# hkust-vgd/scanobjectnn

Hardware: NVIDIA H100
Metric: point-clouds/sec (B=32, N=2048, 15-class) (higher is better)
Workload: dtype f32

## Files before the change

scanobjectnn_b200/csrc/tc_mlp.cu:

```cuda
#include <float.h>
#include <stdlib.h>

#include <atomic>
#include <type_traits>

#include "common.cuh"
#include "mlp_internal.cuh"
#include "tc_common.cuh"

namespace psa {

using namespace tc;

constexpr int kMaxTcLayers = 2;


struct TcArgs {
    long long groups;
    int K;
    int n, m;
    const float* xyz;
    const float* new_xyz;
    const float* uf;
    const int* idx;
// ... 798 lines not shown
                for (int w = 1; w < wpg; ++w) mx = fmaxf(mx, s_red[0][grp * wpg + w][cl]);
                const long long wg = rs / a.pool_k;
                if (!big) {
                    a.out[(size_t)wg * a.N + nt * Nt + cl] = mx;
                } else {
                    int code = __float_as_int(mx);
                    code = code >= 0 ? code : code ^ 0x7fffffff;
                    atomicMax(reinterpret_cast<int*>(a.out) + (size_t)wg * a.N + nt * Nt + cl, code);
                }
            }
            unit_bar_sync(1, kDenseConsumers);
        }
    }
    if constexpr (NP == 2) {
        if (f16x2_overflowed(ovf) || (tid == 0 && a.wflag != nullptr && *a.wflag != 0u)) atomicOr(a.ovf, 1u);
    }
}

bool tc_dense_eligible(long long rows, int K, int N, int pool_k) {
    if (rows < 128 || K < 32 || N < 64 || (N % 64) != 0) return false;
    if (N > 64 && (N % 128) != 0) return false;
    if (!(pool_k == 1 || pool_k == 32 || pool_k == 64 || (pool_k >= 128 && pool_k % 128 == 0))) return false;
    if (pool_k > 1 && rows % pool_k != 0) return false;
    return true;
}

static std::atomic<int> g_tc_np{2};
int tc_np() { return g_tc_np; }

static size_t tc_dense_image_off3(int K, int N) { return tc_image_alloc_bytes((K + 63) & ~63, N, 2); }
size_t tc_dense_image_bytes(int K, int N) { return tc_dense_image_off3(K, N) + tc_image_alloc_bytes((K + 63) & ~63, N, 3); }

static size_t tc_plan_image_bytes(int Kp, int N) { return g_tc_np == 2 ? tc_image_alloc_bytes(Kp, N, 2) + tc_image_alloc_bytes(Kp, N, 3) : tc_image_alloc_bytes(Kp, N, 3); }

int tc_dense_nt(long long rows, int N) {
    const bool wide = (N % 128) == 0 && 2 * ((rows + 127) / 128 * (N / 128)) > kNumSMs;
    return (wide ? 128 : 64) | image_flag(g_tc_np);
}

int build_image(int K, int Kp, int N, int Nt, const float* W, uint8_t* image, cudaStream_t st, const unsigned int* run_if) {
    if (Nt & kImageF16x2) {
        unsigned int* trailer = reinterpret_cast<unsigned int*>(image + tc_image_trailer_off(Kp, N, 2));
        float* colscale = reinterpret_cast<float*>(image + tc_image_colscale_off(Kp, N, 2));
        PSA_CUDA(cudaMemsetAsync(trailer, 0, 256, st));
        tc_col_scale_kernel<<<(N + 31) / 32, dim3(32, 8), 0, st>>>(K, N, W, colscale, trailer);
        int rc = check_launch("tc_col_scale_kernel");
        if (rc != PSA_OK) return rc;
        tc_prep_weights_kernel<2><<<(Kp * N + 255) / 256, 256, 0, st>>>(K, Kp, N, Nt & ~kImageFlags, W, colscale, image, run_if);
    } else {
        tc_prep_weights_kernel<3><<<(Kp * N + 255) / 256, 256, 0, st>>>(K, Kp, N, Nt & ~kImageFlags, W, nullptr, image, run_if);
    }
    return check_launch("tc_prep_weights_kernel");
}
const unsigned int* image_trailer(const uint8_t* image, int Kp, int N) {
    return reinterpret_cast<const unsigned int*>(image + tc_image_trailer_off(Kp, N, 2));
}
const float* image_colscale(const uint8_t* image, int Kp, int N) {
    return reinterpret_cast<const float*>(image + tc_image_colscale_off(Kp, N, 2));
}

template <int NP, int NC>
static int launch_tc_dense_shape(const TcDenseArgs& a, cudaStream_t st) {
    const size_t smem = (size_t)dense_stages(NP, NC) * dense_stage_bytes(NP, NC) + 1024;
    PSA_CUDA(cudaFuncSetAttribute(tc_dense_kernel<NP, NC>, cudaFuncAttributeMaxDynamicSharedMemorySize, (int)smem));
    int dev = 0, sms = 0, per_sm = 0;
    PSA_CUDA(cudaGetDevice(&dev));
    PSA_CUDA(cudaDeviceGetAttribute(&sms, cudaDevAttrMultiProcessorCount, dev));
    PSA_CUDA(cudaOccupancyMaxActiveBlocksPerMultiprocessor(&per_sm, tc_dense_kernel<NP, NC>, kDenseThreads, smem));
    const long long tiles = (a.rows + 127) / 128 * (a.N / (64 * NC)), resident = (long long)sms * (per_sm > 0 ? per_sm : 1);
    tc_dense_kernel<NP, NC><<<(unsigned)(tiles < resident ? tiles : resident), kDenseThreads, smem, st>>>(a);
    return check_launch("tc_dense_kernel");
}

template <int NP>
static int launch_tc_dense_np(TcDenseArgs& a, int Nt, cudaStream_t st) {
    const bool big = a.pool_k > 128;
    if (big) { int rc0 = launch_fill_ord_neg_inf(a.rows / a.pool_k * a.N, a.out, st, a.run_if); if (rc0 != PSA_OK) return rc0; }
    const int rc = Nt == 128 ? launch_tc_dense_shape<NP, 2>(a, st) : launch_tc_dense_shape<NP, 1>(a, st);
    if (rc != PSA_OK) return rc;
    if (big) return launch_decode_ord(a.rows / a.pool_k * a.N, a.out, st, a.run_if);
    return PSA_OK;
}

constexpr int kTileCounterWords = PSA_MAX_MLP_LAYERS;

static int launch_tc_dense_rerun(TcDenseArgs a, int Nt, const float* W, const uint8_t* prebuilt, uint8_t* ws_img, const unsigned int* run_if,
                                 unsigned int* counter, cudaStream_t st) {
    uint8_t* img3 = ws_img + tc_dense_image_off3(a.K, a.N);
    if (prebuilt != nullptr) {
        img3 = const_cast<uint8_t*>(prebuilt) + tc_image_alloc_bytes(a.Kp, a.N, 2);
    } else {
        const int rc = build_image(a.K, a.Kp, a.N, Nt | kImageBf16x3, W, img3, st, run_if);
        if (rc != PSA_OK) return rc;
    }
    a.image = img3; a.ovf = nullptr; a.wflag = nullptr; a.colscale = nullptr; a.run_if = run_if; a.tile_counter = counter;
    return launch_tc_dense_np<3>(a, Nt, st);
}

int launch_tc_dense(long long rows, int K, int N, int pool_k, int relu, const float* x, const float* W, const float* scale,
                    const float* shift, float* out, const uint8_t* prebuilt, uint8_t* ws_img, unsigned int* flag, unsigned int* counters,
                    cudaStream_t st, const float* xyz3 = nullptr, const float* w3 = nullptr, const float* group_add = nullptr,
                    long long group_rows = 0) {
    const int Kp = (K + 63) & ~63;
    const int Nt = tc_dense_nt(rows, N) & ~kImageFlags;
    TcDenseArgs a;
    a.rows = rows; a.K = K; a.Kp = Kp; a.N = N; a.pool_k = pool_k; a.relu = relu;
    a.x = x; a.scale = scale; a.shift = shift; a.out = out; a.xyz3 = xyz3; a.w3 = w3;
    a.group_add = group_add; a.group_rows = group_rows;
    a.tile_counter = counters;
    uint8_t* img3 = ws_img + tc_dense_image_off3(K, N);
    int rc;
    if (g_tc_np == 3) {
        if (prebuilt == nullptr) { rc = build_image(K, Kp, N, Nt | kImageBf16x3, W, img3, st); if (rc != PSA_OK) return rc; }
        a.image = prebuilt ? prebuilt : img3;
        return launch_tc_dense_np<3>(a, Nt, st);
    }
    if (prebuilt == nullptr) { rc = build_image(K, Kp, N, Nt | kImageF16x2, W, ws_img, st); if (rc != PSA_OK) return rc; }
    a.image = prebuilt ? prebuilt : ws_img;
    a.ovf = flag; a.wflag = image_trailer(a.image, Kp, N); a.colscale = image_colscale(a.image, Kp, N);
    rc = launch_tc_dense_np<2>(a, Nt, st);
    if (rc != PSA_OK) return rc;
    return launch_tc_dense_rerun(a, Nt, W, prebuilt, ws_img, flag, counters + 1, st);
}

bool tc_train_fwd_eligible(long long rows, int K, int N) {
    return rows >= 128 && K >= 128 && K <= 512 && N >= 128 && (N % 128) == 0;
}
int launch_tc_dense_train(long long rows, int K, int N, const float* x, const float* in_scale, const float* in_shift, int in_relu,
                          const float* W, const float* bias, float* y, float* stat_partial, uint8_t* image_ws, cudaStream_t st) {
    const int Kp = (K + 63) & ~63;
    int rc = build_image(K, Kp, N, 128 | kImageBf16x3, W, image_ws, st);
    if (rc != PSA_OK) return rc;
    TcDenseArgs a;
    a.rows = rows; a.K = K; a.Kp = Kp; a.N = N; a.pool_k = 1; a.relu = 0;
    a.x = x; a.image = image_ws; a.scale = nullptr; a.shift = bias; a.out = y; a.xyz3 = nullptr; a.w3 = nullptr;
    a.in_scale = in_scale; a.in_shift = in_shift; a.in_relu = in_relu; a.stat_partial = stat_partial;
    return launch_tc_dense_np<3>(a, 128, st);
}

static const uint8_t* prebuilt_image(const psa_mlp* mlp, int l, int row0, int Nt) {
    if (mlp->image[l] != nullptr && mlp->image_nt[l] == Nt && mlp->image_row0[l] == row0) return reinterpret_cast<const uint8_t*>(mlp->image[l]);
    return nullptr;
}

bool tc_sa_eligible(const psa_mlp* mlp, int c, int nsample, TcArgs* out, int np) {
    if (mlp->n_layers < 2 || mlp->n_layers > 1 + kMaxTcLayers) return false;
    if (!(nsample == 32 || nsample == 64 || nsample == 128)) return false;
    if (mlp->channels[0] != 3 + c) return false;
    const int C1 = mlp->channels[1];
    if (!(C1 == 64 || C1 == 128)) return false;
    TcArgs a{};
    a.C1 = C1;
    a.nl = mlp->n_layers - 1;
    a.np = np;
    for (int l = 0; l < a.nl; ++l) {
        a.Kd[l] = mlp->channels[1 + l];
        a.Ntot[l] = mlp->channels[2 + l];
        if (!(a.Kd[l] == 64 || a.Kd[l] == 128)) return false;
        const bool is_last = (l == a.nl - 1);
        if (!is_last && !(a.Ntot[l] == 64 || a.Ntot[l] == 128)) return false;
        if (is_last && !(a.Ntot[l] == 64 || a.Ntot[l] % 128 == 0)) return false;
    }
    a.stream_last = 0;
    if (tc_sa_layout(a).total + 1024 > kSmemBudget) a.stream_last = 1;
    if (tc_sa_layout(a).total + 1024 > kSmemBudget) return false;
    *out = a;
    return true;
}
bool tc_sa_eligible(const psa_mlp* mlp, int c, int nsample, TcArgs* out) {
    TcArgs a3;
    if (!tc_sa_eligible(mlp, c, nsample, &a3, 3)) return false;
    if (g_tc_np == 3) { *out = a3; return true; }
    return tc_sa_eligible(mlp, c, nsample, out, 2);
}

size_t tc_sa_workspace_bytes(const TcArgs& a, int b, int n, int c) {
    size_t bytes = 256;
    for (int l = 0; l < a.nl; ++l) bytes += tc_image_alloc_bytes(a.Kd[l], a.Ntot[l], 2) + tc_image_alloc_bytes(a.Kd[l], a.Ntot[l], 3);
    if (c > 0) bytes += (((size_t)b * n * a.C1 * sizeof(float) + 255) & ~(size_t)255) + tc_dense_image_bytes(c, a.C1);
    return bytes;
}

static int tc_sa_image_nt() { return kSaNt | image_flag(g_tc_np); }

template <int NP, int C1, int NL, int N0>
static int launch_tc_sa_shape(const TcArgs& a, long long ctas_needed, size_t smem, cudaStream_t st) {
    PSA_CUDA(cudaFuncSetAttribute(tc_sa_kernel<NP, C1, NL, N0>, cudaFuncAttributeMaxDynamicSharedMemorySize, (int)smem));
    int dev = 0, sms = 0, per_sm = 0;
    PSA_CUDA(cudaGetDevice(&dev));
    PSA_CUDA(cudaDeviceGetAttribute(&sms, cudaDevAttrMultiProcessorCount, dev));
    PSA_CUDA(cudaOccupancyMaxActiveBlocksPerMultiprocessor(&per_sm, tc_sa_kernel<NP, C1, NL, N0>, kSaThreads, smem));
    const long long resident = (long long)sms * (per_sm > 0 ? per_sm : 1);
    const int ctas = (int)(ctas_needed < 1 ? 1 : ctas_needed < resident ? ctas_needed : resident);
    tc_sa_kernel<NP, C1, NL, N0><<<ctas, kSaThreads, smem, st>>>(a);
    return check_launch("tc_sa_kernel");
}

template <int NP>
static int launch_tc_sa_np(TcArgs& a, cudaStream_t st) {
    const uint32_t limit = 223u * 1024u;
    a.joint = a.K == 128 || a.stream_last;
    if (!a.joint && tc_sa_layout(a).total + 1024 + sa_carry_bytes(a) + sa_red_bytes(1) > limit) a.joint = 1;
    const size_t used = (size_t)tc_sa_layout(a).total + 1024 + sa_carry_bytes(a);
    const int ncl = a.Ntot[a.nl - 1] / 64;
    a.pool_chunks = 1;
    if (!a.stream_last)
        for (int ng = ncl; ng > 1; --ng)
            if (ncl % ng == 0 && used + sa_red_bytes(ng) <= limit) { a.pool_chunks = ng; break; }
    const int C = sa_chunk(a.K, a.joint);
    const long long nchunks = (a.groups + C - 1) / C;
    const long long ctas_needed = a.joint ? nchunks : (nchunks + 1) / 2;
    const size_t smem = used + sa_red_bytes(a.pool_chunks);
    if (a.nl == 1) return a.C1 == 64 ? launch_tc_sa_shape<NP, 64, 1, 0>(a, ctas_needed, smem, st) : launch_tc_sa_shape<NP, 128, 1, 0>(a, ctas_needed, smem, st);
    if (a.C1 == 64) return a.Ntot[0] == 64 ? launch_tc_sa_shape<NP, 64, 2, 64>(a, ctas_needed, smem, st) : launch_tc_sa_shape<NP, 64, 2, 128>(a, ctas_needed, smem, st);
    return a.Ntot[0] == 64 ? launch_tc_sa_shape<NP, 128, 2, 64>(a, ctas_needed, smem, st) : launch_tc_sa_shape<NP, 128, 2, 128>(a, ctas_needed, smem, st);
}

static int tc_sa_run(TcArgs& a, int b, int n, int m, int c, int nsample, const float* xyz, const float* new_xyz, const float* points,
                     const int* idx, const psa_mlp* mlp, const float* w1c, float* out, void* workspace, cudaStream_t st) {
    int rc = PSA_OK;
    uint8_t* ws = reinterpret_cast<uint8_t*>(workspace);
    unsigned int* words = reinterpret_cast<unsigned int*>(ws);
    PSA_CUDA(cudaMemsetAsync(ws, 0, 256, st));
    ws += 256;
    uint8_t* img2[kMaxTcLayers];
    uint8_t* img3[kMaxTcLayers];
    for (int l = 0; l < a.nl; ++l) {
        img2[l] = ws; ws += tc_image_alloc_bytes(a.Kd[l], a.Ntot[l], 2);
        img3[l] = ws; ws += tc_image_alloc_bytes(a.Kd[l], a.Ntot[l], 3);
    }
    const float* uf = nullptr;
    if (c > 0) {
        float* ufw = reinterpret_cast<float*>(ws);
        uint8_t* uimg = ws + (((size_t)b * n * a.C1 * sizeof(float) + 255) & ~(size_t)255);
        const float* w1f = mlp->weight[0] + (size_t)3 * a.C1;
        if (tc_dense_eligible((long long)b * n, c, a.C1, 1)) {
            rc = launch_tc_dense((long long)b * n, c, a.C1, 1, 0, points, w1f, nullptr, nullptr, ufw, prebuilt_image(mlp, 0, 3, tc_dense_nt((long long)b * n, a.C1)),
                                 uimg, words + 3, words + 4, st);
        } else {
            DenseArgs d;
            d.rows = (long long)b * n; d.K = c; d.N = a.C1; d.pool_k = 1; d.relu = 0;
            d.x = points; d.W = w1f; d.scale = nullptr; d.shift = nullptr; d.out = ufw;
            rc = launch_dense(d, st);
        }
        if (rc != PSA_OK) return rc;
        uf = ufw;
    }
    auto fill = [&](TcArgs& t) {
        t.groups = (long long)b * m; t.K = nsample; t.n = n; t.m = m;
        t.xyz = xyz; t.new_xyz = new_xyz; t.idx = idx; t.out = out; t.uf = uf;
        t.w1x = mlp->weight[0]; t.s1 = mlp->scale[0]; t.t1 = mlp->shift[0]; t.relu1 = mlp->relu[0];
        t.ovf = nullptr; t.run_if = nullptr; t.w1c = w1c;
        for (int l = 0; l < t.nl; ++l) {
            t.s[l] = mlp->scale[1 + l]; t.t[l] = mlp->shift[1 + l]; t.relu[l] = mlp->relu[1 + l]; t.wflag[l] = nullptr; t.colscale[l] = nullptr;
        }
    };
    fill(a);
    for (int l = 0; l < a.nl; ++l) {
        const int nt_img = tc_sa_image_nt();
        const uint8_t* pre = prebuilt_image(mlp, 1 + l, 0, nt_img);
        uint8_t* own = a.np == 2 ? img2[l] : img3[l];
        if (pre == nullptr) { rc = build_image(a.Kd[l], a.Kd[l], a.Ntot[l], nt_img, mlp->weight[1 + l], own, st); if (rc != PSA_OK) return rc; }
        a.image[l] = pre ? pre : own;
        if (a.np == 2) { a.wflag[l] = image_trailer(a.image[l], a.Kd[l], a.Ntot[l]); a.colscale[l] = image_colscale(a.image[l], a.Kd[l], a.Ntot[l]); }
    }
    a.tile_counter = words;
    if (a.np == 3) return launch_tc_sa_np<3>(a, st);
    a.ovf = words + 2;
    rc = launch_tc_sa_np<2>(a, st);
    if (rc != PSA_OK) return rc;
    TcArgs a3;
    PSA_REQUIRE(tc_sa_eligible(mlp, c, nsample, &a3, 3), "sa_module: internal error (bf16x3 eligibility)");
    fill(a3);
    for (int l = 0; l < a3.nl; ++l) {
        const uint8_t* pre = prebuilt_image(mlp, 1 + l, 0, kSaNt | kImageF16x2);
        if (pre != nullptr) {
            a3.image[l] = pre + tc_image_alloc_bytes(a3.Kd[l], a3.Ntot[l], 2);
        } else {
            rc = build_image(a3.Kd[l], a3.Kd[l], a3.Ntot[l], kSaNt | kImageBf16x3, mlp->weight[1 + l], img3[l], st, words + 2);
            if (rc != PSA_OK) return rc;
            a3.image[l] = img3[l];
        }
    }
    a3.tile_counter = words + 1;
    a3.run_if = words + 2;
    return launch_tc_sa_np<3>(a3, st);
}

struct TcGroupAllArgs {
    int c;
    int N[3];
    int Nt[3];
    const float* points;
    const float* xyz;
    const float* w3;
    const uint8_t* image[3];
    const float* colscale[3];
    const unsigned int* wflag[3];
    const float* scale[3];
    const float* shift[3];
    int relu[3];
    float* out;
    unsigned int* ovf;
};

constexpr int kGaStages = 3;
constexpr uint32_t kGaStageBytes = 32768u;
constexpr uint32_t kGaSmemBudget = 222u * 1024u;
__host__ __device__ inline uint32_t group_all_smem(int W0, int W1, int W2) {
    return 1024u + kGaStages * kGaStageBytes + (uint32_t)(W0 + W1) / 64u * kDenseXBytes + 12u * (uint32_t)(W0 + W1 + W2);
}

__device__ __forceinline__ uint32_t cluster_ctarank() {
    uint32_t r;
    asm volatile("mov.u32 %0, %%cluster_ctarank;\n" : "=r"(r));
    return r;
}
__device__ __forceinline__ uint32_t mapa_shared(uint32_t addr, uint32_t rank) {
    uint32_t r;
    asm volatile("mapa.shared::cluster.u32 %0, %1, %2;\n" : "=r"(r) : "r"(addr), "r"(rank));
    return r;
}
__device__ __forceinline__ float2 ld_cluster_f32x2(uint32_t addr) {
    float2 v;
    asm volatile("ld.shared::cluster.v2.f32 {%0, %1}, [%2];\n" : "=f"(v.x), "=f"(v.y) : "r"(addr) : "memory");
    return v;
}
__device__ __forceinline__ void cluster_sync_all() {
    asm volatile("barrier.cluster.arrive.release.aligned;\n\tbarrier.cluster.wait.acquire.aligned;\n" ::: "memory");
}
__device__ __forceinline__ void mbar_arrive_cluster(uint32_t addr) {
    asm volatile("fence.acq_rel.cluster;\n\tmbarrier.arrive.release.cluster.shared::cluster.b64 _, [%0];\n" ::"r"(addr) : "memory");
}
__device__ __forceinline__ void mbar_wait_cluster(uint64_t* bar, uint32_t parity) {
    uint32_t done;
    const uint32_t addr = smem_u32(bar);
    do {
        asm volatile(
            "{\n\t.reg .pred p;\n\t"
            "mbarrier.try_wait.parity.acquire.cluster.shared::cta.b64 p, [%1], %2;\n\t"
            "selp.u32 %0, 1, 0, p;\n\t}\n"
            : "=r"(done)
            : "r"(addr), "r"(parity)
            : "memory");
    } while (!done);
}

template <int NC0, int NC1>
__global__ void __cluster_dims__(4, 1, 1) __launch_bounds__(kDenseThreads, 1)
tc_group_all_kernel(const __grid_constant__ TcGroupAllArgs a) {
    constexpr int NP = 2, S = kGaStages;
    constexpr uint32_t piece = 8192u, chunk = 16384u;
    extern __shared__ uint8_t smem_raw[];
    __shared__ __align__(8) uint64_t s_full[S], s_empty[S], s_ready[2], s_done;
    __shared__ float s_red[8][128];
    const int tid = threadIdx.x, lane = tid & 31, warp = tid >> 5;
    const uint32_t rank = cluster_ctarank();
    const int cloud = blockIdx.x >> 2;
    uint8_t* base = smem_raw + ((1024u - (smem_u32(smem_raw) & 1023u)) & 1023u);
    constexpr int W0 = 64 * NC0, W1 = 64 * NC1;
    const int W2 = a.N[2] / 4;
    uint8_t* slice0 = base + S * kGaStageBytes;
    uint8_t* slice1 = slice0 + NC0 * kDenseXBytes;
    float* aff0 = reinterpret_cast<float*>(slice1 + NC1 * kDenseXBytes);
    float* aff1 = aff0 + 3 * W0;
    float* aff2 = aff1 + 3 * W1;
    {
        float* aff[3] = {aff0, aff1, aff2};
        const int W[3] = {W0, W1, W2};
#pragma unroll
        for (int l = 0; l < 3; ++l)
            for (int i = tid; i < W[l]; i += kDenseThreads) {
                const int col = (int)rank * W[l] + i;
                const float cs = __ldg(a.colscale[l] + col);
                aff[l][i] = (a.scale[l] ? __ldg(a.scale[l] + col) : 1.f) * cs;
                aff[l][W[l] + i] = a.shift[l] ? __ldg(a.shift[l] + col) : 0.f;
                aff[l][2 * W[l] + i] = pow2_rcp(cs);
            }
    }
    if (tid == 0) {
        for (int i = 0; i < S; ++i) { mbar_init(&s_full[i], 1); mbar_init(&s_empty[i], kDenseConsumers / 32); }
        mbar_init(&s_ready[0], 4); mbar_init(&s_ready[1], 4); mbar_init(&s_done, 4);
        fence_mbar_init();
    }
    __syncthreads();
    cluster_sync_all();
    const int KC[3] = {a.c / 64, 4 * W0 / 64, 4 * W1 / 64};

    if (warp >= kDenseConsumers / 32) {
        asm volatile("setmaxnreg.dec.sync.aligned.u32 40;\n");
        if (warp != kDenseConsumers / 32) return;
        uint32_t u = 0;
#pragma unroll
        for (int l = 0; l < 3; ++l) {
            const int pw = l == 0 ? W0 : l == 1 ? W1 : 128, passes = l == 2 ? W2 / 128 : 1, Nt = a.Nt[l];
            for (int p = 0; p < passes; ++p) {
                const int j0 = ((int)rank * (l == 0 ? W0 : l == 1 ? W1 : W2) + p * pw) / 64;
                for (int kb = 0; kb < KC[l]; ++kb, ++u) {
                    const int s = (int)(u % S);
                    if (u >= (uint32_t)S) mbar_wait(&s_empty[s], ((u / S) - 1u) & 1u);
                    if (lane == 0) {
                        mbar_expect_tx(&s_full[s], (uint32_t)(pw / 64) * chunk);
                        for (int c = 0; c < pw / 64; ++c) {
                            uint8_t* dst = base + (uint32_t)s * kGaStageBytes + (uint32_t)c * chunk;
                            const int j = j0 + c;
                            if (Nt == 64) {
                                bulk_g2s(dst, a.image[l] + ((size_t)j * KC[l] + kb) * chunk, chunk, &s_full[s]);
                            } else {
                                const uint8_t* src = a.image[l] + ((size_t)(j >> 1) * KC[l] + kb) * (2u * chunk) + (uint32_t)(j & 1) * piece;
                                bulk_g2s(dst, src, piece, &s_full[s]);
                                bulk_g2s(dst + piece, src + 2u * piece, piece, &s_full[s]);
                            }
                        }
                    }
                }
            }
        }
        return;
    }

    asm volatile("setmaxnreg.inc.sync.aligned.u32 232;\n");
    const int g = lane >> 2, t = lane & 3;
    const int rl[2] = {warp * 16 + g, warp * 16 + g + 8};
    uint32_t ovf = 0u;
    uint32_t u = 0;

    auto pass = [&](auto Ltag, auto NCtag, int lc) {
        constexpr int L = decltype(Ltag)::value, NC = decltype(NCtag)::value;
        const int nkb = KC[L];
        auto prep = [&](uint32_t (&A)[NP][4][4], int kb) {
            if constexpr (L == 0) {
                const float* xb = a.points + (size_t)cloud * 128 * a.c + kb * 64;
#pragma unroll
                for (int s = 0; s < 4; ++s)
#pragma unroll
                    for (int h = 0; h < 2; ++h)
#pragma unroll
                        for (int i = 0; i < 2; ++i) {
                            const float2 x = __ldg(reinterpret_cast<const float2*>(xb + (size_t)rl[i] * a.c + 16 * s + 8 * h + 2 * t));
                            put_a<NP, 4>(A, s, i + 2 * h, x.x, x.y, ovf);
                        }
            } else {
                constexpr int Wp = L == 1 ? W0 : W1;
                const uint32_t src = mapa_shared(smem_u32(L == 1 ? slice0 : slice1) + (uint32_t)((kb * 64) % Wp / 64) * kDenseXBytes,
                                                 (uint32_t)(kb * 64 / Wp));
#pragma unroll
                for (int s = 0; s < 4; ++s)
#pragma unroll
                    for (int h = 0; h < 2; ++h)
#pragma unroll
                        for (int i = 0; i < 2; ++i) {
                            const float2 x = ld_cluster_f32x2(src + (uint32_t)rl[i] * kDenseXRow + (uint32_t)(16 * s + 8 * h + 2 * t) * 4u);
                            put_a<NP, 4>(A, s, i + 2 * h, x.x, x.y, ovf);
                        }
            }
        };
        float acc[NC][32];
        auto step = [&](const uint32_t (&A)[NP][4][4], uint32_t (&An)[NP][4][4], int kb) {
            const int s = (int)(u % S);
            mbar_wait(&s_full[s], (u / S) & 1u);
            const uint32_t wb = smem_u32(base) + (uint32_t)s * kGaStageBytes;
            float d[NC][32];
            wg_fence();
#pragma unroll
            for (int tt = 0; tt < Split<NP>::kTerms; ++tt)
#pragma unroll
                for (int ks = 0; ks < 4; ++ks)
#pragma unroll
                    for (int c = 0; c < NC; ++c)
                        wg_mma_rs<NP>(d[c], A[Split<NP>::a(tt)][ks][0], A[Split<NP>::a(tt)][ks][1], A[Split<NP>::a(tt)][ks][2], A[Split<NP>::a(tt)][ks][3],
                                      wg_desc(wb + (uint32_t)c * chunk + Split<NP>::w(tt) * piece + (uint32_t)ks * 32u), (tt | ks) ? 1u : 0u);
            wg_commit();
            if (kb + 1 < nkb) prep(An, kb + 1);
            wg_wait_all();
            __syncwarp();
            if (lane == 0) mbar_arrive1(&s_empty[s]);
            ++u;
#pragma unroll
            for (int c = 0; c < NC; ++c) {
                wg_fence_acc(d[c]);
#pragma unroll
                for (int e = 0; e < 32; ++e) acc[c][e] = kb ? acc[c][e] + d[c][e] : d[c][e];
            }
        };
        {
            uint32_t A0[NP][4][4], A1[NP][4][4];
            prep(A0, 0);
            for (int kb = 0;; kb += 2) {
                step(A0, A1, kb);
                if (kb + 1 == nkb) break;
                step(A1, A0, kb + 1);
                if (kb + 2 == nkb) break;
            }
        }

        constexpr int W = L == 0 ? W0 : L == 1 ? W1 : 0;
        const int Wl = L == 2 ? W2 : W;
        const float* aff = L == 0 ? aff0 : L == 1 ? aff1 : aff2;
        float xs[2][3] = {{0.f, 0.f, 0.f}, {0.f, 0.f, 0.f}};
        if constexpr (L == 0)
#pragma unroll
            for (int i = 0; i < 2; ++i)
#pragma unroll
                for (int k = 0; k < 3; ++k) xs[i][k] = __ldg(a.xyz + ((size_t)cloud * 128 + rl[i]) * 3 + k);
#pragma unroll
        for (int c = 0; c < NC; ++c)
#pragma unroll
            for (int j = 0; j < 8; ++j) {
                const int cl = c * 64 + 8 * j + 2 * t, ls = lc + cl;
                float y[2][2];
#pragma unroll
                for (int e = 0; e < 2; ++e) {
                    const float sc = aff[ls + e], sh = aff[Wl + ls + e];
                    float w0 = 0.f, w1 = 0.f, w2 = 0.f;
                    if constexpr (L == 0) {
                        const int col = (int)rank * W0 + ls + e;
                        const float f = aff[2 * Wl + ls + e];
                        w0 = __ldg(a.w3 + col) * f; w1 = __ldg(a.w3 + a.N[0] + col) * f; w2 = __ldg(a.w3 + 2 * a.N[0] + col) * f;
                    }
#pragma unroll
                    for (int i = 0; i < 2; ++i) {
                        float x = acc[c][4 * j + 2 * i + e];
                        if constexpr (L == 0) x = fmaf(xs[i][2], w2, fmaf(xs[i][1], w1, fmaf(xs[i][0], w0, x)));
                        x = fmaf(x, sc, sh);
                        if (a.relu[L]) x = fmaxf(x, 0.f);
                        y[i][e] = x;
                    }
                }
                if constexpr (L < 2) {
                    uint8_t* sl = (L == 0 ? slice0 : slice1) + (ls >> 6) * kDenseXBytes + (ls & 63) * 4;
#pragma unroll
                    for (int i = 0; i < 2; ++i) *reinterpret_cast<float2*>(sl + rl[i] * kDenseXRow) = make_float2(y[i][0], y[i][1]);
                } else {
#pragma unroll
                    for (int e = 0; e < 2; ++e) {
                        const float m = warp_rowmax16(y[0][e], y[1][e]);
                        if (g == 0) s_red[warp][cl + e] = m;
                    }
                }
            }
        unit_bar_sync(1, kDenseConsumers);
        if constexpr (L < 2) {
            if (tid < 4) mbar_arrive_cluster(mapa_shared(smem_u32(&s_ready[L]), (uint32_t)tid));
            mbar_wait_cluster(&s_ready[L], 0);
        } else {
            for (int cl = tid; cl < 64 * NC; cl += kDenseConsumers) {
                float mx = s_red[0][cl];
                for (int w = 1; w < 8; ++w) mx = fmaxf(mx, s_red[w][cl]);
                a.out[(size_t)cloud * a.N[2] + (size_t)rank * W2 + lc + cl] = mx;
            }
            unit_bar_sync(1, kDenseConsumers);
        }
    };
    pass(std::integral_constant<int, 0>{}, std::integral_constant<int, NC0>{}, 0);
    pass(std::integral_constant<int, 1>{}, std::integral_constant<int, NC1>{}, 0);
    for (int lc = 0; lc < W2; lc += 128) pass(std::integral_constant<int, 2>{}, std::integral_constant<int, 2>{}, lc);

    if (tid < 4) mbar_arrive_cluster(mapa_shared(smem_u32(&s_done), (uint32_t)tid));
    if (f16x2_overflowed(ovf) || (tid == 0 && (*a.wflag[0] | *a.wflag[1] | *a.wflag[2]) != 0u)) atomicOr(a.ovf, 1u);
    mbar_wait_cluster(&s_done, 0);
}

template <int NC0, int NC1>
static size_t group_all_fits(const psa_mlp* mlp) {
    const size_t smem = group_all_smem(64 * NC0, 64 * NC1, mlp->channels[3] / 4);
    if (smem > kGaSmemBudget) return 0;
    if (cudaFuncSetAttribute(tc_group_all_kernel<NC0, NC1>, cudaFuncAttributeMaxDynamicSharedMemorySize, (int)smem) != cudaSuccess) return 0;
    cudaLaunchConfig_t cfg = {};
    cfg.gridDim = dim3(4, 1, 1);
    cfg.blockDim = dim3(kDenseThreads, 1, 1);
    cfg.dynamicSmemBytes = smem;
    int clusters = 0;
    if (cudaOccupancyMaxActiveClusters(&clusters, tc_group_all_kernel<NC0, NC1>, &cfg) != cudaSuccess) { (void)cudaGetLastError(); return 0; }
    return clusters > 0 ? smem : 0;
}
static size_t group_all_eligible(int n, int c, const float* points, const psa_mlp* mlp) {
    if (g_tc_np != 2 || mlp->n_layers != 3 || n != 128 || c < 64 || c % 64 != 0 || (reinterpret_cast<uintptr_t>(points) & 15) != 0) return 0;
    const int N0 = mlp->channels[1], N1 = mlp->channels[2], N2 = mlp->channels[3];
    if (N2 % 512 != 0) return 0;
    if (N0 == 256 && N1 == 256) return group_all_fits<1, 1>(mlp);
    if (N0 == 256 && N1 == 512) return group_all_fits<1, 2>(mlp);
    if (N0 == 512 && N1 == 256) return group_all_fits<2, 1>(mlp);
    return 0;
}

static int sa_group_all_cluster(int b, int c, const float* xyz, const float* points, const psa_mlp* mlp, float* out, float* ws0, float* ws1,
                                uint8_t* img, unsigned int* words, size_t smem, cudaStream_t st) {
    const long long rows = (long long)b * 128;
    unsigned int* flag = words + kTileCounterWords - 1;
    TcGroupAllArgs g{};
    g.c = c; g.points = points; g.xyz = xyz; g.w3 = mlp->weight[0]; g.out = out; g.ovf = flag;
    const uint8_t* pre[3];
    uint8_t* ws_img[3];
    int rc;
    for (int l = 0; l < 3; ++l) {
        const int K = l == 0 ? c : mlp->channels[l], N = mlp->channels[l + 1], Nt = tc_dense_nt(rows, N);
        const float* W = l == 0 ? mlp->weight[0] + (size_t)3 * N : mlp->weight[l];
        pre[l] = prebuilt_image(mlp, l, l == 0 ? 3 : 0, Nt);
        ws_img[l] = img;
        img += tc_dense_image_bytes(K, N);
        if (pre[l] == nullptr) { rc = build_image(K, K, N, Nt, W, ws_img[l], st); if (rc != PSA_OK) return rc; }
        const uint8_t* image = pre[l] ? pre[l] : ws_img[l];
        g.N[l] = N; g.Nt[l] = Nt & ~kImageFlags; g.image[l] = image;
        g.colscale[l] = image_colscale(image, K, N); g.wflag[l] = image_trailer(image, K, N);
        g.scale[l] = mlp->scale[l]; g.shift[l] = mlp->shift[l]; g.relu[l] = mlp->relu[l];
    }
    const int N0 = mlp->channels[1], N1 = mlp->channels[2];
    if (N0 == 256 && N1 == 256) tc_group_all_kernel<1, 1><<<4u * (unsigned)b, kDenseThreads, smem, st>>>(g);
    else if (N0 == 256) tc_group_all_kernel<1, 2><<<4u * (unsigned)b, kDenseThreads, smem, st>>>(g);
    else tc_group_all_kernel<2, 1><<<4u * (unsigned)b, kDenseThreads, smem, st>>>(g);
    rc = check_launch("tc_group_all_kernel");
    if (rc != PSA_OK) return rc;
    const float* cur = points;
    for (int l = 0; l < 3; ++l) {
        const int K = l == 0 ? c : mlp->channels[l], N = mlp->channels[l + 1];
        TcDenseArgs a;
        a.rows = rows; a.K = K; a.Kp = K; a.N = N; a.pool_k = l == 2 ? 128 : 1; a.relu = mlp->relu[l];
        a.x = cur; a.scale = mlp->scale[l]; a.shift = mlp->shift[l]; a.out = l == 2 ? out : (l & 1) ? ws1 : ws0;
        a.xyz3 = l == 0 ? xyz : nullptr; a.w3 = l == 0 ? mlp->weight[0] : nullptr;
        rc = launch_tc_dense_rerun(a, g.Nt[l], l == 0 ? mlp->weight[0] + (size_t)3 * N : mlp->weight[l], pre[l], ws_img[l], flag,
                                   words + kTileCounterWords + 2 * l + 1, st);
        if (rc != PSA_OK) return rc;
        cur = a.out;
    }
    return PSA_OK;
}

}

using namespace psa;

static std::atomic<int> g_mlp_mode{0};
int psa::mlp_mode() { return g_mlp_mode; }
extern "C" PSA_API int psa_set_mlp_mode(int mode) {
    PSA_REQUIRE(mode == 0 || mode == 1 || mode == 2,
                "set_mlp_mode: mode must be 0 (tensor cores, fp16x2 operands with the range guard), 1 (fp32 FMA kernels only) or 2 (tensor cores, bf16x3)");
    g_mlp_mode = mode;
    g_tc_np = mode == 2 ? 3 : 2;
    return PSA_OK;
}
extern "C" PSA_API int psa_get_mlp_mode(void) { return g_mlp_mode; }

extern "C" size_t psa_sa_module_workspace_bytes(int b, int n, int m, int c, int nsample, const psa_mlp* mlp) {
    (void)m;
    TcArgs a;
    if (g_mlp_mode != 1 && mlp != nullptr && tc_sa_eligible(mlp, c, nsample, &a)) return tc_sa_workspace_bytes(a, b, n, c);
    return 0;
}

extern "C" int psa_sa_module_infer(int b, int n, int m, int c, float radius, int nsample, const float* xyz,
                                   const float* new_xyz, const float* points, const int* idx_in, const psa_mlp* mlp,
                                   float* out, int* idx_out, int* pts_cnt, void* workspace, size_t workspace_bytes,
                                   psa_stream_t stream) {
    int rc = validate_mlp_public(mlp, "sa_module");
    if (rc != PSA_OK) return rc;
    PSA_REQUIRE(b >= 0 && n >= 1 && m >= 0 && c >= 0 && nsample >= 1, "sa_module: bad dims b=%d n=%d m=%d c=%d nsample=%d", b, n, m, c, nsample);
    PSA_REQUIRE(mlp->channels[0] == 3 + c, "sa_module: mlp input width %d != 3 + c (%d)", mlp->channels[0], 3 + c);
    if (b == 0 || m == 0) return PSA_OK;
    PSA_REQUIRE(xyz && new_xyz && out && (points || c == 0), "sa_module: null buffer");
    const int* idx = idx_in;
    if (idx == nullptr) {
        PSA_REQUIRE(idx_out != nullptr, "sa_module: idx_out must be provided when idx_in is NULL (it receives the ball query)");
        rc = psa_query_ball_point(b, n, m, radius, nsample, xyz, new_xyz, idx_out, pts_cnt, stream);
        if (rc != PSA_OK) return rc;
        idx = idx_out;
    }
    cudaStream_t st = as_stream(stream);
    TcArgs a;
    if (g_mlp_mode != 1 && tc_sa_eligible(mlp, c, nsample, &a)) {
        const size_t need = tc_sa_workspace_bytes(a, b, n, c);
        PSA_REQUIRE(workspace != nullptr && workspace_bytes >= need,
                    "sa_module: workspace of %zu bytes required (psa_sa_module_workspace_bytes), got %zu", need, workspace_bytes);
        PSA_REQUIRE((reinterpret_cast<uintptr_t>(workspace) & 255) == 0, "sa_module: workspace must be 256-byte aligned");
        return tc_sa_run(a, b, n, m, c, nsample, xyz, new_xyz, points, idx, mlp, nullptr, out, workspace, st);
    }
    return sa_module_simt(b, n, m, c, nsample, xyz, new_xyz, points, idx, mlp, out, st);
}

extern "C" size_t psa_shared_mlp_workspace_bytes(long long rows, const psa_mlp* mlp) {
    if (mlp == nullptr || mlp->n_layers < 1) return 0;
    size_t bytes = 0;
    int cmax = 0;
    for (int l = 1; l < mlp->n_layers; ++l) cmax = cmax > mlp->channels[l] ? cmax : mlp->channels[l];
    if (mlp->n_layers > 1) bytes += 2 * (((size_t)rows * cmax * sizeof(float) + 255) & ~(size_t)255);
    for (int l = 0; l < mlp->n_layers; ++l) bytes += tc_dense_image_bytes(mlp->channels[l], mlp->channels[l + 1] < 64 ? 64 : mlp->channels[l + 1]);
    if (rows <= 32) {
        size_t fc = 0;
        for (int l = 0; l < mlp->n_layers; ++l) { size_t f = fc_small_workspace_bytes(mlp->channels[l], mlp->channels[l + 1]); fc = f > fc ? f : fc; }
        bytes += (fc + 255) & ~(size_t)255;
    }
    return bytes + 256;
}

static int shared_mlp_chain(long long rows, int pool_k, const float* x, const psa_mlp* mlp, const float* group_add, long long group_rows,
                            float* out, void* workspace, size_t workspace_bytes, psa_stream_t stream) {
    int rc;
    const int L = mlp->n_layers;
    const size_t need = psa_shared_mlp_workspace_bytes(rows, mlp);
    PSA_REQUIRE(workspace != nullptr && workspace_bytes >= need, "shared_mlp: workspace of %zu bytes required (got %zu)", need, workspace_bytes);
    PSA_REQUIRE((reinterpret_cast<uintptr_t>(workspace) & 255) == 0, "shared_mlp: workspace must be 256-byte aligned");
    int cmax = 0;
    for (int l = 1; l < L; ++l) cmax = cmax > mlp->channels[l] ? cmax : mlp->channels[l];
    const size_t half = L > 1 ? (((size_t)rows * cmax * sizeof(float) + 255) & ~(size_t)255) : 0;
    uint8_t* wsb = reinterpret_cast<uint8_t*>(workspace);
    float* ws0 = reinterpret_cast<float*>(wsb);
    float* ws1 = reinterpret_cast<float*>(wsb + half);
    uint8_t* img = wsb + 2 * half;
    float* fc_partial = nullptr;
    if (rows <= 32) {
        size_t imgs = 0;
        for (int l = 0; l < L; ++l) imgs += tc_dense_image_bytes(mlp->channels[l], mlp->channels[l + 1] < 64 ? 64 : mlp->channels[l + 1]);
        fc_partial = reinterpret_cast<float*>(img + imgs);
    }
    const float* cur = x;
    cudaStream_t st = as_stream(stream);
    unsigned int* flags = reinterpret_cast<unsigned int*>(wsb + need - 256);
    PSA_CUDA(cudaMemsetAsync(flags, 0, 256, st));
    for (int l = 0; l < L; ++l) {
        const int K = mlp->channels[l], N = mlp->channels[l + 1];
        const int pk = (l == L - 1) ? pool_k : 1;
        float* dst = (l == L - 1) ? out : ((l & 1) ? ws1 : ws0);
        const float* gadd = l == 0 ? group_add : nullptr;
        if (g_mlp_mode != 1 && tc_dense_eligible(rows, K, N, pk)) {
            rc = launch_tc_dense(rows, K, N, pk, mlp->relu[l], cur, mlp->weight[l], mlp->scale[l], mlp->shift[l], dst, prebuilt_image(mlp, l, 0, tc_dense_nt(rows, N)),
                                 img, flags + l, flags + kTileCounterWords + 2 * l, st, nullptr, nullptr, gadd, group_rows);
        } else {
            DenseArgs d;
            d.rows = rows; d.K = K; d.N = N; d.pool_k = pk; d.relu = mlp->relu[l];
            d.x = cur; d.W = mlp->weight[l]; d.scale = mlp->scale[l]; d.shift = mlp->shift[l]; d.out = dst;
            d.group_add = gadd; d.group_rows = group_rows;
            rc = (rows <= 32 && pk == 1 && gadd == nullptr) ? launch_fc_small(d, fc_partial, st) : launch_dense(d, st);
        }
        if (rc != PSA_OK) return rc;
        img += tc_dense_image_bytes(K, N < 64 ? 64 : N);
        cur = dst;
    }
    return PSA_OK;
}

extern "C" int psa_shared_mlp(long long rows, int pool_k, const float* x, const psa_mlp* mlp, float* out,
                              void* workspace, size_t workspace_bytes, psa_stream_t stream) {
    int rc = validate_mlp_public(mlp, "shared_mlp");
    if (rc != PSA_OK) return rc;
    PSA_REQUIRE(rows >= 0 && pool_k >= 1, "shared_mlp: rows=%lld pool_k=%d", rows, pool_k);
    if (rows == 0) return PSA_OK;
    PSA_REQUIRE(rows % pool_k == 0, "shared_mlp: rows=%lld is not a multiple of pool_k=%d", rows, pool_k);
    PSA_REQUIRE(x && out, "shared_mlp: null buffer");
    return shared_mlp_chain(rows, pool_k, x, mlp, nullptr, 0, out, workspace, workspace_bytes, stream);
}

extern "C" int psa_shared_mlp_grouped(long long rows, long long group_rows, const float* x, const psa_mlp* mlp, const float* group_add,
                                      float* out, void* workspace, size_t workspace_bytes, psa_stream_t stream) {
    int rc = validate_mlp_public(mlp, "shared_mlp_grouped");
    if (rc != PSA_OK) return rc;
    PSA_REQUIRE(rows >= 0 && group_rows >= 1, "shared_mlp_grouped: rows=%lld group_rows=%lld", rows, group_rows);
    PSA_REQUIRE(rows % group_rows == 0, "shared_mlp_grouped: group_rows=%lld does not divide rows=%lld", group_rows, rows);
    if (rows == 0) return PSA_OK;
    PSA_REQUIRE(x && group_add && out, "shared_mlp_grouped: null buffer");
    return shared_mlp_chain(rows, 1, x, mlp, group_add, group_rows, out, workspace, workspace_bytes, stream);
}

extern "C" size_t psa_sa_group_all_workspace_bytes(int b, int n, int c, const psa_mlp* mlp) {
    if (mlp == nullptr || mlp->n_layers < 1) return 0;
    psa_mlp m2 = *mlp;
    m2.channels[0] = c;
    return psa_shared_mlp_workspace_bytes((long long)b * n, &m2);
}

extern "C" int psa_sa_group_all_infer(int b, int n, int c, const float* xyz, const float* points, const psa_mlp* mlp,
                                      float* out, void* workspace, size_t workspace_bytes, psa_stream_t stream) {
    int rc = validate_mlp_public(mlp, "sa_group_all");
    if (rc != PSA_OK) return rc;
    PSA_REQUIRE(b >= 0 && n >= 1 && c >= 1, "sa_group_all: bad dims b=%d n=%d c=%d", b, n, c);
    PSA_REQUIRE(mlp->channels[0] == 3 + c, "sa_group_all: mlp input width %d != 3 + c (%d)", mlp->channels[0], 3 + c);
    if (b == 0) return PSA_OK;
    PSA_REQUIRE(xyz && points && out, "sa_group_all: null buffer");
    const long long rows = (long long)b * n;
    const int L = mlp->n_layers;
    const int N0 = mlp->channels[1];
    const int pk0 = (L == 1) ? n : 1;
    PSA_SUPPORTED(g_mlp_mode != 1 && tc_dense_eligible(rows, c, N0, pk0),
                  "sa_group_all: first layer (%d -> %d over %lld rows) is not eligible for the tensor-core path; concatenate and use shared_mlp", c, N0, rows);
    const size_t need = psa_sa_group_all_workspace_bytes(b, n, c, mlp);
    PSA_REQUIRE(workspace != nullptr && workspace_bytes >= need, "sa_group_all: workspace of %zu bytes required (got %zu)", need, workspace_bytes);
    PSA_REQUIRE((reinterpret_cast<uintptr_t>(workspace) & 255) == 0, "sa_group_all: workspace must be 256-byte aligned");
    int cmax = 0;
    for (int l = 1; l < L; ++l) cmax = cmax > mlp->channels[l] ? cmax : mlp->channels[l];
    const size_t half = L > 1 ? (((size_t)rows * cmax * sizeof(float) + 255) & ~(size_t)255) : 0;
    uint8_t* wsb = reinterpret_cast<uint8_t*>(workspace);
    float* ws0 = reinterpret_cast<float*>(wsb);
    float* ws1 = reinterpret_cast<float*>(wsb + half);
    uint8_t* img = wsb + 2 * half;
    cudaStream_t st = as_stream(stream);
    unsigned int* flags = reinterpret_cast<unsigned int*>(wsb + need - 256);
    PSA_CUDA(cudaMemsetAsync(flags, 0, 256, st));
    if (g_mlp_mode == 0) {
        const size_t smem = group_all_eligible(n, c, points, mlp);
        if (smem != 0) return sa_group_all_cluster(b, c, xyz, points, mlp, out, ws0, ws1, img, flags, smem, st);
    }
    const float* cur = points;
    for (int l = 0; l < L; ++l) {
        const int K = (l == 0) ? c : mlp->channels[l], N = mlp->channels[l + 1];
        const int pk = (l == L - 1) ? n : 1;
        float* dst = (l == L - 1) ? out : ((l & 1) ? ws1 : ws0);
        const float* W = (l == 0) ? mlp->weight[0] + (size_t)3 * N : mlp->weight[l];
        if (tc_dense_eligible(rows, K, N, pk)) {
            rc = launch_tc_dense(rows, K, N, pk, mlp->relu[l], cur, W, mlp->scale[l], mlp->shift[l], dst, prebuilt_image(mlp, l, l == 0 ? 3 : 0, tc_dense_nt(rows, N)),
                                 img, flags + l, flags + kTileCounterWords + 2 * l, st, l == 0 ? xyz : nullptr, l == 0 ? mlp->weight[0] : nullptr);
        } else {
            PSA_SUPPORTED(l > 0, "sa_group_all: layer 0 must run on the tensor-core path");
            DenseArgs d;
            d.rows = rows; d.K = K; d.N = N; d.pool_k = pk; d.relu = mlp->relu[l];
            d.x = cur; d.W = W; d.scale = mlp->scale[l]; d.shift = mlp->shift[l]; d.out = dst;
            rc = launch_dense(d, st);
        }
        if (rc != PSA_OK) return rc;
        img += tc_dense_image_bytes(K, N < 64 ? 64 : N);
        cur = dst;
    }
    return PSA_OK;
}

__global__ void edge_wc_kernel(int c, int N, const float* __restrict__ W, float* __restrict__ Wc) {
    const int total = c * 2 * N;
    for (int e = blockIdx.x * blockDim.x + threadIdx.x; e < total; e += gridDim.x * blockDim.x) {
        const int kk = e / (2 * N), j = e - kk * 2 * N;
        Wc[e] = j < N ? __ldg(W + (size_t)kk * N + j) - __ldg(W + (size_t)(c + kk) * N + j) : __ldg(W + (size_t)(c + kk) * N + j - N);
    }
}

template <int VEC>
__global__ void __launch_bounds__(256)
edge_gather_max_kernel(long long points, int n, int k, int N, const float* __restrict__ AB, const int* __restrict__ nn_idx,
                       const float* __restrict__ scale, const float* __restrict__ shift, int relu, float* __restrict__ out) {
    const int lane = threadIdx.x & 31;
    const long long warp0 = (long long)blockIdx.x * 8 + (threadIdx.x >> 5);
    float sc[VEC], sh[VEC];
#pragma unroll
    for (int v = 0; v < VEC; ++v) {
        sc[v] = scale ? __ldg(scale + lane * VEC + v) : 1.f;
        sh[v] = shift ? __ldg(shift + lane * VEC + v) : 0.f;
    }
    for (long long p = warp0; p < points; p += (long long)gridDim.x * 8) {
        const long long base = (p / n) * n;
        const float* arow = AB + (size_t)p * 2 * N + lane * VEC;
        float a[VEC], mx[VEC], mn[VEC];
#pragma unroll
        for (int v = 0; v < VEC; ++v) { a[v] = __ldg(arow + v); mx[v] = -FLT_MAX; mn[v] = FLT_MAX; }
        const int myj = lane < k ? __ldg(nn_idx + p * k + lane) : 0;
        for (int j = 0; j < k; ++j) {
            const int nb = __shfl_sync(0xffffffffu, myj, j);
            const float* brow = AB + (size_t)(base + nb) * 2 * N + N + lane * VEC;
#pragma unroll
            for (int v = 0; v < VEC; ++v) { const float bv = __ldg(brow + v); mx[v] = fmaxf(mx[v], bv); mn[v] = fminf(mn[v], bv); }
        }
#pragma unroll
        for (int v = 0; v < VEC; ++v) {
            float y = fmaf(a[v] + (sc[v] >= 0.f ? mx[v] : mn[v]), sc[v], sh[v]);
            if (relu) y = fmaxf(y, 0.f);
            out[(size_t)p * N + lane * VEC + v] = y;
        }
    }
}

static bool edgeconv_algebra_ok(long long rows, int c, int k, const psa_mlp* mlp) {
    const int N = mlp->channels[1];
    return g_mlp_mode != 1 && mlp->n_layers == 1 && rows >= 128 && k <= 32 && (N == 32 || N == 64 || N == 128 || N == 256) && c >= 1;
}

__global__ void edge_pad_idx_kernel(long long rows, int k, const int* __restrict__ idx, int* __restrict__ idx32) {
    for (long long e = (long long)blockIdx.x * blockDim.x + threadIdx.x; e < rows * 32; e += (long long)gridDim.x * blockDim.x) {
        const long long r = e >> 5;
        const int j = (int)(e & 31);
        idx32[e] = __ldg(idx + r * k + (j < k ? j : 0));
    }
}
static bool edgeconv_dual_ok(int c, int k, const psa_mlp* mlp, psa_mlp* m2, TcArgs* a) {
    if (g_mlp_mode == 1 || c != 3 || k < 1 || k > 32 || mlp->n_layers < 2) return false;
    *m2 = *mlp;
    m2->channels[0] = 3;
    m2->weight[0] = mlp->weight[0] + (size_t)3 * mlp->channels[1];
    for (int l = 0; l < PSA_MAX_MLP_LAYERS; ++l) { m2->image[l] = nullptr; m2->image_nt[l] = 0; m2->image_row0[l] = 0; }
    return tc_sa_eligible(m2, 0, 32, a);
}

extern "C" size_t psa_edgeconv_workspace_bytes(int b, int n, int c, int k, const psa_mlp* mlp) {
    if (mlp == nullptr) return 0;
    const long long rows = (long long)b * n;
    {
        psa_mlp m2;
        TcArgs a;
        if (edgeconv_dual_ok(c, k, mlp, &m2, &a)) return (((size_t)rows * 32 * 4 + 255) & ~(size_t)255) + tc_sa_workspace_bytes(a, b, n, 0);
    }
    if (!edgeconv_algebra_ok(rows, c, k, mlp)) return 0;
    const int N = mlp->channels[1];
    return (((size_t)c * 2 * N * 4 + 255) & ~(size_t)255) + (((size_t)rows * 2 * N * 4 + 255) & ~(size_t)255) + tc_dense_image_bytes(c, 2 * N) + 256;
}

extern "C" int psa_edgeconv_infer(int b, int n, int c, int k, const float* x, const int* nn_idx, const psa_mlp* mlp,
                                  float* out, void* workspace, size_t workspace_bytes, psa_stream_t stream) {
    int rc = validate_mlp_public(mlp, "edgeconv");
    if (rc != PSA_OK) return rc;
    PSA_REQUIRE(b >= 0 && n >= 0 && c >= 1 && k >= 1, "edgeconv: bad dims b=%d n=%d c=%d k=%d", b, n, c, k);
    PSA_REQUIRE(mlp->channels[0] == 2 * c, "edgeconv: mlp input width %d != 2*c (%d)", mlp->channels[0], 2 * c);
    if (b == 0 || n == 0) return PSA_OK;
    PSA_REQUIRE(x && nn_idx && out, "edgeconv: null buffer");
    cudaStream_t st = as_stream(stream);
    const long long rows = (long long)b * n;
    {
        psa_mlp m2;
        TcArgs a;
        if (edgeconv_dual_ok(c, k, mlp, &m2, &a)) {
            const size_t need = psa_edgeconv_workspace_bytes(b, n, c, k, mlp);
            PSA_REQUIRE(workspace != nullptr && workspace_bytes >= need, "edgeconv: workspace of %zu bytes required (got %zu)", need, workspace_bytes);
            PSA_REQUIRE((reinterpret_cast<uintptr_t>(workspace) & 255) == 0, "edgeconv: workspace must be 256-byte aligned");
            int* idx32 = reinterpret_cast<int*>(workspace);
            edge_pad_idx_kernel<<<(unsigned)((rows * 32 + 255) / 256 < 65535 * 4 ? (rows * 32 + 255) / 256 : 65535 * 4), 256, 0, st>>>(rows, k, nn_idx, idx32);
            rc = check_launch("edge_pad_idx_kernel");
            if (rc != PSA_OK) return rc;
            return tc_sa_run(a, b, n, n, 0, 32, x, x, nullptr, idx32, &m2, mlp->weight[0], out,
                             reinterpret_cast<uint8_t*>(workspace) + (((size_t)rows * 32 * 4 + 255) & ~(size_t)255), st);
        }
    }
    if (!edgeconv_algebra_ok(rows, c, k, mlp)) return edgeconv_simt(b, n, c, k, x, nn_idx, mlp, out, st);
    const int N = mlp->channels[1];
    const size_t need = psa_edgeconv_workspace_bytes(b, n, c, k, mlp);
    PSA_REQUIRE(workspace != nullptr && workspace_bytes >= need, "edgeconv: workspace of %zu bytes required (got %zu)", need, workspace_bytes);
    PSA_REQUIRE((reinterpret_cast<uintptr_t>(workspace) & 255) == 0, "edgeconv: workspace must be 256-byte aligned");
    uint8_t* ws = reinterpret_cast<uint8_t*>(workspace);
    float* Wc = reinterpret_cast<float*>(ws);
    ws += ((size_t)c * 2 * N * 4 + 255) & ~(size_t)255;
    float* AB = reinterpret_cast<float*>(ws);
    ws += ((size_t)rows * 2 * N * 4 + 255) & ~(size_t)255;
    edge_wc_kernel<<<(c * 2 * N + 255) / 256, 256, 0, st>>>(c, N, mlp->weight[0], Wc);
    if (tc_dense_eligible(rows, c, 2 * N, 1)) {
        unsigned int* flag = reinterpret_cast<unsigned int*>(reinterpret_cast<uint8_t*>(workspace) + need - 256);
        PSA_CUDA(cudaMemsetAsync(flag, 0, 256, st));
        rc = launch_tc_dense(rows, c, 2 * N, 1, 0, x, Wc, nullptr, nullptr, AB, nullptr, ws, flag, flag + 1, st);
    } else {
        DenseArgs d;
        d.rows = rows; d.K = c; d.N = 2 * N; d.pool_k = 1; d.relu = 0;
        d.x = x; d.W = Wc; d.scale = nullptr; d.shift = nullptr; d.out = AB;
        rc = launch_dense(d, st);
    }
// ... 45 lines not shown
```

Baseline: 93570.

## Prefetch next A tile before barrier wait and vectorize cluster slice loads

In the fused group-all kernel, the next k-block's activations are now loaded into registers before waiting on the weight stage, and converted to split-precision fragments after the MMAs are issued. Global loads and DSMEM reads therefore overlap the barrier wait and the MMA. Cluster-shared slice reads go from 2-float to 4-float vector loads, using a permuted column layout (ga_slice_col) that the epilogue store also follows. Register limits move from 40/232 to 24/240 for producer/consumer, and optional compile-time timing instrumentation is added. The extra live registers for the prefetched tile risk spills.

```diff
diff --git a/scanobjectnn_b200/csrc/tc_mlp.cu b/scanobjectnn_b200/csrc/tc_mlp.cu
--- a/scanobjectnn_b200/csrc/tc_mlp.cu
+++ b/scanobjectnn_b200/csrc/tc_mlp.cu
@@ -1124,7 +1124,25 @@
     int relu[3];
     float* out;
     unsigned int* ovf;
+#ifdef PSA_GA_TIMING
+    unsigned long long* timing;
+#endif
 };
+
+#ifdef PSA_GA_TIMING
+constexpr int kGaTimingWords = 28;
+static unsigned long long* g_ga_timing = nullptr;
+#define GA_MARK(L, PH)                                                                                     \
+    do {                                                                                                   \
+        const long long now_ = clock64();                                                                  \
+        if (lane == 0) atomicAdd(&s_t[(L) * 8 + (PH)], (unsigned long long)(now_ - t_mark));              \
+        t_mark = now_;                                                                                     \
+    } while (0)
+#else
+#define GA_MARK(L, PH) \
+    do {               \
+    } while (0)
+#endif
 
 constexpr int kGaStages = 3;
 constexpr uint32_t kGaStageBytes = 32768u;
@@ -1143,11 +1161,19 @@
     asm volatile("mapa.shared::cluster.u32 %0, %1, %2;\n" : "=r"(r) : "r"(addr), "r"(rank));
     return r;
 }
-__device__ __forceinline__ float2 ld_cluster_f32x2(uint32_t addr) {
-    float2 v;
-    asm volatile("ld.shared::cluster.v2.f32 {%0, %1}, [%2];\n" : "=f"(v.x), "=f"(v.y) : "r"(addr) : "memory");
-    return v;
-}
+__device__ __forceinline__ void ld_cluster_row4(uint32_t addr, float2 (&v)[4][2]) {
+    asm volatile(
+        "ld.shared::cluster.v4.f32 {%0, %1, %2, %3}, [%16];\n\t"
+        "ld.shared::cluster.v4.f32 {%4, %5, %6, %7}, [%16+64];\n\t"
+        "ld.shared::cluster.v4.f32 {%8, %9, %10, %11}, [%16+128];\n\t"
+        "ld.shared::cluster.v4.f32 {%12, %13, %14, %15}, [%16+192];\n"
+        : "=f"(v[0][0].x), "=f"(v[0][0].y), "=f"(v[0][1].x), "=f"(v[0][1].y), "=f"(v[1][0].x), "=f"(v[1][0].y), "=f"(v[1][1].x),
+          "=f"(v[1][1].y), "=f"(v[2][0].x), "=f"(v[2][0].y), "=f"(v[2][1].x), "=f"(v[2][1].y), "=f"(v[3][0].x), "=f"(v[3][0].y),
+          "=f"(v[3][1].x), "=f"(v[3][1].y)
+        : "r"(addr)
+        : "memory");
+}
+__host__ __device__ constexpr int ga_slice_col(int q) { return (q & ~15) + 4 * ((q & 7) >> 1) + 2 * ((q >> 3) & 1) + (q & 1); }
 __device__ __forceinline__ void cluster_sync_all() {
     asm volatile("barrier.cluster.arrive.release.aligned;\n\tbarrier.cluster.wait.acquire.aligned;\n" ::: "memory");
 }
@@ -1177,6 +1203,12 @@
     __shared__ __align__(8) uint64_t s_full[S], s_empty[S], s_ready[2], s_done;
     __shared__ float s_red[8][128];
     const int tid = threadIdx.x, lane = tid & 31, warp = tid >> 5;
+#ifdef PSA_GA_TIMING
+    const long long t_start = clock64();
+    long long t_mark = t_start;
+    __shared__ unsigned long long s_t[24];
+    if (tid < 24) s_t[tid] = 0ull;
+#endif
     const uint32_t rank = cluster_ctarank();
     const int cloud = blockIdx.x >> 2;
     uint8_t* base = smem_raw + ((1024u - (smem_u32(smem_raw) & 1023u)) & 1023u);
@@ -1210,7 +1242,7 @@
     const int KC[3] = {a.c / 64, 4 * W0 / 64, 4 * W1 / 64};
 
     if (warp >= kDenseConsumers / 32) {
-        asm volatile("setmaxnreg.dec.sync.aligned.u32 40;\n");
+        asm volatile("setmaxnreg.dec.sync.aligned.u32 24;\n");
         if (warp != kDenseConsumers / 32) return;
         uint32_t u = 0;
 #pragma unroll
@@ -1220,7 +1252,13 @@
                 const int j0 = ((int)rank * (l == 0 ? W0 : l == 1 ? W1 : W2) + p * pw) / 64;
                 for (int kb = 0; kb < KC[l]; ++kb, ++u) {
                     const int s = (int)(u % S);
+#ifdef PSA_GA_TIMING
+                    const long long t0 = clock64();
+#endif
                     if (u >= (uint32_t)S) mbar_wait(&s_empty[s], ((u / S) - 1u) & 1u);
+#ifdef PSA_GA_TIMING
+                    if (lane == 0 && a.timing) atomicAdd(a.timing + 24 + l, (unsigned long long)(clock64() - t0));
+#endif
                     if (lane == 0) {
                         mbar_expect_tx(&s_full[s], (uint32_t)(pw / 64) * chunk);
                         for (int c = 0; c < pw / 64; ++c) {
@@ -1238,49 +1276,56 @@
                 }
             }
         }
+#ifdef PSA_GA_TIMING
+        if (lane == 0 && a.timing) atomicAdd(a.timing + 27, (unsigned long long)(clock64() - t_start));
+#endif
         return;
     }
 
-    asm volatile("setmaxnreg.inc.sync.aligned.u32 232;\n");
+    asm volatile("setmaxnreg.inc.sync.aligned.u32 240;\n");
     const int g = lane >> 2, t = lane & 3;
     const int rl[2] = {warp * 16 + g, warp * 16 + g + 8};
     uint32_t ovf = 0u;
     uint32_t u = 0;
+    GA_MARK(0, 7);
 
     auto pass = [&](auto Ltag, auto NCtag, int lc) {
         constexpr int L = decltype(Ltag)::value, NC = decltype(NCtag)::value;
         const int nkb = KC[L];
-        auto prep = [&](uint32_t (&A)[NP][4][4], int kb) {
+        auto load = [&](float2 (&R)[2][4][2], int kb) {
             if constexpr (L == 0) {
                 const float* xb = a.points + (size_t)cloud * 128 * a.c + kb * 64;
 #pragma unroll
-                for (int s = 0; s < 4; ++s)
-#pragma unroll
-                    for (int h = 0; h < 2; ++h)
-#pragma unroll
-                        for (int i = 0; i < 2; ++i) {
-                            const float2 x = __ldg(reinterpret_cast<const float2*>(xb + (size_t)rl[i] * a.c + 16 * s + 8 * h + 2 * t));
-                            put_a<NP, 4>(A, s, i + 2 * h, x.x, x.y, ovf);
-                        }
+                for (int i = 0; i < 2; ++i)
+#pragma unroll
+                    for (int s = 0; s < 4; ++s)
+#pragma unroll
+                        for (int h = 0; h < 2; ++h)
+                            R[i][s][h] = __ldg(reinterpret_cast<const float2*>(xb + (size_t)rl[i] * a.c + 16 * s + 8 * h + 2 * t));
             } else {
                 constexpr int Wp = L == 1 ? W0 : W1;
                 const uint32_t src = mapa_shared(smem_u32(L == 1 ? slice0 : slice1) + (uint32_t)((kb * 64) % Wp / 64) * kDenseXBytes,
                                                  (uint32_t)(kb * 64 / Wp));
 #pragma unroll
-                for (int s = 0; s < 4; ++s)
-#pragma unroll
-                    for (int h = 0; h < 2; ++h)
-#pragma unroll
-                        for (int i = 0; i < 2; ++i) {
-                            const float2 x = ld_cluster_f32x2(src + (uint32_t)rl[i] * kDenseXRow + (uint32_t)(16 * s + 8 * h + 2 * t) * 4u);
-                            put_a<NP, 4>(A, s, i + 2 * h, x.x, x.y, ovf);
-                        }
-            }
+                for (int i = 0; i < 2; ++i) ld_cluster_row4(src + (uint32_t)rl[i] * kDenseXRow + (uint32_t)ga_slice_col(2 * t) * 4u, R[i]);
+            }
+        };
+        auto split = [&](uint32_t (&A)[NP][4][4], const float2 (&R)[2][4][2]) {
+#pragma unroll
+            for (int s = 0; s < 4; ++s)
+#pragma unroll
+                for (int h = 0; h < 2; ++h)
+#pragma unroll
+                    for (int i = 0; i < 2; ++i) put_a<NP, 4>(A, s, i + 2 * h, R[i][s][h].x, R[i][s][h].y, ovf);
         };
         float acc[NC][32];
         auto step = [&](const uint32_t (&A)[NP][4][4], uint32_t (&An)[NP][4][4], int kb) {
             const int s = (int)(u % S);
+            float2 R[2][4][2];
+            if (kb + 1 < nkb) load(R, kb + 1);
+            GA_MARK(L, 2);
             mbar_wait(&s_full[s], (u / S) & 1u);
+            GA_MARK(L, 0);
             const uint32_t wb = smem_u32(base) + (uint32_t)s * kGaStageBytes;
             float d[NC][32];
             wg_fence();
@@ -1293,8 +1338,11 @@
                         wg_mma_rs<NP>(d[c], A[Split<NP>::a(tt)][ks][0], A[Split<NP>::a(tt)][ks][1], A[Split<NP>::a(tt)][ks][2], A[Split<NP>::a(tt)][ks][3],
                                       wg_desc(wb + (uint32_t)c * chunk + Split<NP>::w(tt) * piece + (uint32_t)ks * 32u), (tt | ks) ? 1u : 0u);
             wg_commit();
-            if (kb + 1 < nkb) prep(An, kb + 1);
+            GA_MARK(L, 1);
+            if (kb + 1 < nkb) split(An, R);
+            GA_MARK(L, 2);
             wg_wait_all();
+            GA_MARK(L, 3);
             __syncwarp();
             if (lane == 0) mbar_arrive1(&s_empty[s]);
             ++u;
@@ -1304,10 +1352,16 @@
 #pragma unroll
                 for (int e = 0; e < 32; ++e) acc[c][e] = kb ? acc[c][e] + d[c][e] : d[c][e];
             }
+            GA_MARK(L, 4);
         };
         {
             uint32_t A0[NP][4][4], A1[NP][4][4];
-            prep(A0, 0);
+            {
+                float2 R[2][4][2];
+                load(R, 0);
+                split(A0, R);
+            }
+            GA_MARK(L, 2);
             for (int kb = 0;; kb += 2) {
                 step(A0, A1, kb);
                 if (kb + 1 == nkb) break;
@@ -1350,7 +1404,7 @@
                     }
                 }
                 if constexpr (L < 2) {
-                    uint8_t* sl = (L == 0 ? slice0 : slice1) + (ls >> 6) * kDenseXBytes + (ls & 63) * 4;
+                    uint8_t* sl = (L == 0 ? slice0 : slice1) + (ls >> 6) * kDenseXBytes + ga_slice_col(ls & 63) * 4;
 #pragma unroll
                     for (int i = 0; i < 2; ++i) *reinterpret_cast<float2*>(sl + rl[i] * kDenseXRow) = make_float2(y[i][0], y[i][1]);
                 } else {
@@ -1364,7 +1418,9 @@
         unit_bar_sync(1, kDenseConsumers);
         if constexpr (L < 2) {
             if (tid < 4) mbar_arrive_cluster(mapa_shared(smem_u32(&s_ready[L]), (uint32_t)tid));
+            GA_MARK(L, 5);
             mbar_wait_cluster(&s_ready[L], 0);
+            GA_MARK(L, 6);
         } else {
             for (int cl = tid; cl < 64 * NC; cl += kDenseConsumers) {
                 float mx = s_red[0][cl];
@@ -1372,6 +1428,7 @@
                 a.out[(size_t)cloud * a.N[2] + (size_t)rank * W2 + lc + cl] = mx;
             }
             unit_bar_sync(1, kDenseConsumers);
+            GA_MARK(L, 5);
         }
     };
     pass(std::integral_constant<int, 0>{}, std::integral_constant<int, NC0>{}, 0);
@@ -1380,8 +1437,15 @@
 
     if (tid < 4) mbar_arrive_cluster(mapa_shared(smem_u32(&s_done), (uint32_t)tid));
     if (f16x2_overflowed(ovf) || (tid == 0 && (*a.wflag[0] | *a.wflag[1] | *a.wflag[2]) != 0u)) atomicOr(a.ovf, 1u);
+    GA_MARK(2, 5);
     mbar_wait_cluster(&s_done, 0);
-}
+#ifdef PSA_GA_TIMING
+    GA_MARK(2, 6);
+    unit_bar_sync(1, kDenseConsumers);
+    if (tid < 24 && a.timing) atomicAdd(a.timing + tid, s_t[tid]);
+#endif
+}
+#undef GA_MARK
 
 template <int NC0, int NC1>
 static size_t group_all_fits(const psa_mlp* mlp) {
@@ -1412,6 +1476,9 @@
     unsigned int* flag = words + kTileCounterWords - 1;
     TcGroupAllArgs g{};
     g.c = c; g.points = points; g.xyz = xyz; g.w3 = mlp->weight[0]; g.out = out; g.ovf = flag;
+#ifdef PSA_GA_TIMING
+    g.timing = g_ga_timing;
+#endif
     const uint8_t* pre[3];
     uint8_t* ws_img[3];
     int rc;
@@ -1462,6 +1529,12 @@
     return PSA_OK;
 }
 extern "C" PSA_API int psa_get_mlp_mode(void) { return g_mlp_mode; }
+#ifdef PSA_GA_TIMING
+extern "C" PSA_API int psa_ga_timing_buffer(void* counters) {
+    g_ga_timing = static_cast<unsigned long long*>(counters);
+    return kGaTimingWords;
+}
+#endif
 
 extern "C" size_t psa_sa_module_workspace_bytes(int b, int n, int m, int c, int nsample, const psa_mlp* mlp) {
     (void)m;
```

Result: no change. 95580, median of 6 (+2.2%).
